# Borda/pyImSegm

Hardware: AMD Instinct MI355X
Metric: Mpixels/s end-to-end SLIC+fts+GC, 2048x2048 RGB; % HBM roofline (higher is better)
Workload: dtype f64; 1 GPU; single 2048x2048 RGB uint8 per GPU, SLIC(sp_size=46, K=2025, 10 sweeps) + colour mean/std/energy + 3-class alpha-expansion GC (gc_regul=2.0, edge=model), pre-fitted GMM, host numpy in -> segm int32 in host numpy (BASELINE configs[1]); bench_config=2, images_per_launch_chain=1, images_in_flight_per_gpu=4, hardware_queues=4, input_memory=pageable numpy, input_ring=default (one rank: measured in round 4), parallelism=images sharded over 1 GPU(s), 4 in flight per GPU (one HIP stream each)

## Files before the change

include/imsegm_hip.h:

```cpp
#ifndef IMSEGM_HIP_H
#define IMSEGM_HIP_H

#include <stddef.h>
#include <stdint.h>

#ifdef __cplusplus
extern "C" {
#endif

#define IMSEGM_API __attribute__((visibility("default")))

#define IMSEGM_U8 0
#define IMSEGM_F64 1
#define IMSEGM_F32 2

#define IMSEGM_E_FUSED_PATH (-3)

#define IMSEGM_E_FIT_CAPS (-4)

typedef struct imsegm_ctx imsegm_ctx;
typedef struct imsegm_image2d imsegm_image2d;

IMSEGM_API const char *imsegm_last_error(void);
IMSEGM_API int imsegm_version(void);
// ... 23 lines not shown
IMSEGM_API int imsegm_image2d_create(imsegm_ctx *ctx, int height, int width, imsegm_image2d **img_out);
IMSEGM_API void imsegm_image2d_destroy(imsegm_image2d *img);

IMSEGM_API int imsegm_image2d_upload(imsegm_image2d *img, const void *host_pixels, int dtype);

IMSEGM_API int imsegm_image2d_slic(imsegm_image2d *img, int minmax_normalize, int n_segments, double compactness,
                        const double *taps_z, int radius_z, const double *taps_y, int radius_y,
                        const double *taps_x, int radius_x, int max_iter, int enforce_connectivity,
                        double min_size_factor, double max_size_factor, int start_label,
                        int max_candidates, int slic_zero, int *n_labels_out);

IMSEGM_API int imsegm_image2d_get_labels(imsegm_image2d *img, int64_t *labels_out);
IMSEGM_API int imsegm_image2d_set_labels(imsegm_image2d *img, const int32_t *labels, int n_labels);
IMSEGM_API long imsegm_debug_conn_general_runs(void);
IMSEGM_API int imsegm_debug_slic_sweep_runs(long *persistent_runs_out, long *fallback_runs_out);
IMSEGM_API long imsegm_debug_gc_grid_fallbacks(void);
IMSEGM_API int imsegm_debug_exclusive_scan(const int32_t *host_in, int n, int32_t *host_out, int32_t *total);
IMSEGM_API int imsegm_image2d_enforce_connectivity(imsegm_image2d *img, const int32_t *labels, long min_size, long max_size,
                                                   int start_label, int *n_labels_out);
IMSEGM_API int imsegm_image2d_label_hist(imsegm_image2d *img, const int32_t *annot, int nb_annot, int64_t *hist_out);
IMSEGM_API int imsegm_image2d_get_lab(imsegm_image2d *img, double *lab_out);
IMSEGM_API int imsegm_image2d_get_nearest(imsegm_image2d *img, int32_t *nearest_out);
IMSEGM_API int imsegm_image2d_get_pre_scalars(imsegm_image2d *img, double out[3]);

IMSEGM_API int imsegm_image2d_color_stats(imsegm_image2d *img, double *mean_out, double *energy_out, double *var_out);

IMSEGM_API int imsegm_image2d_graph(imsegm_image2d *img, int32_t *edges_out, int edge_capacity, int *n_edges_out,
                         double *centres_out, uint8_t *present_out);

IMSEGM_API int imsegm_image2d_gather(imsegm_image2d *img, const int32_t *graph_labels, const double *proba,
// ... 219 lines not shown
```

pyimsegm_amd/_hip.py:

```python
import ctypes as C
import functools
import os
import threading

import numpy as np

_HERE = os.path.dirname(os.path.abspath(__file__))
LIB_PATH = os.environ.get('IMSEGM_HIP_LIBRARY') or os.path.join(_HERE, 'libimsegm_hip.so')

U8, F64, F32 = 0, 1, 2
PROFILE_GROUPS = {
    'slic_assign': 0,
    'slic': 1,
    'connectivity': 2,
    'color_stats': 3,
    'graph': 4,
    'graphcut': 5,
    'gather': 6,
    'slic_preprocess': 7,
    'terms': 8,
    'texture': 9,
}


# ... 68 lines not shown
    'imsegm_ctx_destroy': (None, [_vp]),
    'imsegm_ctx_synchronize': (C.c_int, [_vp]),
    'imsegm_ctx_profile_enable': (C.c_int, [_vp, C.c_int]),
    'imsegm_ctx_profile_reset': (C.c_int, [_vp]),
    'imsegm_ctx_profile_get': (C.c_int, [_vp, C.c_int, C.POINTER(C.c_double), _ip]),
    'imsegm_image2d_create': (C.c_int, [_vp, C.c_int, C.c_int, C.POINTER(_vp)]),
    'imsegm_image2d_destroy': (None, [_vp]),
    'imsegm_image2d_upload': (C.c_int, [_vp, _vp, C.c_int]),
    'imsegm_image2d_slic': (C.c_int, [_vp, C.c_int, C.c_int, C.c_double, _vp, C.c_int, _vp, C.c_int, _vp, C.c_int,
                                      C.c_int, C.c_int, C.c_double, C.c_double, C.c_int, C.c_int, C.c_int, _ip]),
    'imsegm_image2d_get_labels': (C.c_int, [_vp, _vp]),
    'imsegm_image2d_set_labels': (C.c_int, [_vp, _vp, C.c_int]),
    'imsegm_image2d_enforce_connectivity': (C.c_int, [_vp, _vp, C.c_long, C.c_long, C.c_int, _vp]),
    'imsegm_debug_conn_general_runs': (C.c_long, []),
    'imsegm_debug_slic_sweep_runs': (C.c_int, [_vp, _vp]),
    'imsegm_debug_gc_grid_fallbacks': (C.c_long, []),
    'imsegm_debug_exclusive_scan': (C.c_int, [_vp, C.c_int, _vp, _ip]),
    'imsegm_assume_bg_on_boundary': (C.c_int, [_vp, _vp, C.c_int, C.c_int, _vp, C.c_int, _ip]),
    'imsegm_image2d_all_finite': (C.c_int, [_vp, _ip]),
    'imsegm_image2d_lm_features': (C.c_int, [_vp, _vp, _vp, C.c_int, C.c_int, C.c_double, C.c_int, _vp]),
    'imsegm_batch2d_create': (C.c_int, [_vp, C.c_int, C.c_int, C.c_int, C.POINTER(_vp)]),
    'imsegm_batch2d_destroy': (None, [_vp]),
    'imsegm_batch2d_run_color': (C.c_int, [_vp, C.c_int, _vp, C.c_int, C.c_int, C.c_int, C.c_double, _vp, C.c_int, C.c_int, C.c_int,
                                           C.c_int, _vp, C.c_int, _vp, C.c_int, C.c_double, C.c_int, _vp, _vp, _vp]),
    'imsegm_batch2d_device_ptr': (C.c_int, [_vp, C.c_int, C.c_int, C.POINTER(_vp)]),
    'imsegm_device_pci_bus_id': (C.c_int, [C.c_int, C.c_char_p, C.c_int]),
    'imsegm_init': (C.c_int, [C.c_int]),
    'imsegm_debug_reload_env': (None, []),
    'imsegm_image2d_label_hist': (C.c_int, [_vp, _vp, C.c_int, _vp]),
    'imsegm_image2d_get_lab': (C.c_int, [_vp, _vp]),
# ... 1161 lines not shown


def exclusive_scan(values):
    values = np.ascontiguousarray(values, dtype=np.int32)
    out, total = np.empty_like(values), C.c_int(0)
    _check(load_library().imsegm_debug_exclusive_scan(values.ctypes.data, values.size, out.ctypes.data, C.byref(total)))
    return out, total.value


def slic_sweep_runs():
    a, b = C.c_long(0), C.c_long(0)
    _check(load_library().imsegm_debug_slic_sweep_runs(C.byref(a), C.byref(b)))
    return a.value, b.value


def assign_sweeps_per_launch(max_iter=10):
    persistent, fallback = slic_sweep_runs()
    return max_iter - 1 if (persistent > 0 and fallback == 0) else 1


def _device_array(sess, which, shape, typestr):
    ptr = _vp()
    _check(load_library().imsegm_image2d_device_ptr(sess._h, which, C.byref(ptr)))
    sess.ctx.synchronize()
    return DeviceArray(ptr.value, shape, typestr, sess)


def segm_device_array(sess):
    return _device_array(sess, 1, sess.shape, '<i4')

# ... 406 lines not shown
```

pyimsegm_amd/csrc/api.hip:

```cpp
#include "../../include/imsegm_hip.h"
#include "slic.h"

#include <atomic>
#include <cstdio>
#include <cstdlib>
#include <cstring>
#include <vector>

namespace imsegm {

static thread_local std::string g_error;

void set_error(const std::string &msg) { g_error = msg; }

bool hip_ok(hipError_t e, const char *what, const char *file, int line)
{
    if (e == hipSuccess) return true;
    char buf[512];
    snprintf(buf, sizeof(buf), "HIP error %d (%s) in `%s` at %s:%d", (int)e, hipGetErrorString(e), what, file, line);
    g_error = buf;
    return false;
}

static Knobs read_knobs()
{
    auto flag = [](const char *n) { return getenv(n) != nullptr; };
    auto num = [](const char *n, int dflt) { const char *e = getenv(n); return e ? atoi(e) : dflt; };
    Knobs k;
    k.slic_graph = flag("IMSEGM_SLIC_GRAPH");
    k.pre_3pass = flag("IMSEGM_PRE_3PASS");
    k.separate_finalize = flag("IMSEGM_SEPARATE_FINALIZE");
    k.fuse_finalize = flag("IMSEGM_FUSE_FINALIZE");
    k.conn_general = flag("IMSEGM_CONN_GENERAL");
    k.gc_no_topo_regs = flag("IMSEGM_GC_NO_TOPO_REGS");
    k.sep_wide_tile = flag("IMSEGM_SEP_WIDE_TILE");
    k.cc_merge_full = flag("IMSEGM_CC_MERGE_FULL");
    k.label_general = flag("IMSEGM_LABEL_GENERAL");
    k.terms_one_workgroup = flag("IMSEGM_TERMS_ONE_WORKGROUP");
    k.adjacency_table = flag("IMSEGM_ADJACENCY_TABLE");
    k.brick_cap = num("IMSEGM_BRICK_CAP", 0);
    k.gc_lds_level = num("IMSEGM_GC_LDS_LEVEL", 4);
    k.gc_threads = num("IMSEGM_GC_THREADS", 0);
    k.gc_grid_min_sites = num("IMSEGM_GC_GRID_MIN_SITES", 0);
    k.gc_grid_blocks = num("IMSEGM_GC_GRID_BLOCKS", 0);
    k.gc_one_workgroup = flag("IMSEGM_GC_ONE_WORKGROUP");
    k.gc_grid_test_absent = flag("IMSEGM_GC_GRID_TEST_ABSENT");
    k.fused_bitmap_mb = num("IMSEGM_FUSED_BITMAP_MB", 0);
// ... 252 lines not shown
    return 0;
}

long imsegm_debug_conn_general_runs(void) { return conn_general_runs(); }

void imsegm_debug_reload_env(void) { reload_knobs(); }

long imsegm_debug_gc_grid_fallbacks(void) { return gc_grid_fallbacks(); }

int imsegm_debug_slic_sweep_runs(long *persistent_runs_out, long *fallback_runs_out)
{
    slic_sweep_counters(persistent_runs_out, fallback_runs_out);
    return 0;
}

int imsegm_debug_exclusive_scan(const int32_t *host_in, int n, int32_t *host_out, int32_t *total)
{
    if (n < 0 || !total || (n > 0 && (!host_in || !host_out))) {
        set_error("exclusive_scan: n >= 0, and no null pointers");
        return -1;
    }
    int32_t *dev = nullptr;
    HIP_TRY(hipMalloc(&dev, ((size_t)n + 1) * sizeof(int32_t)));
    hipError_t e = n ? hipMemcpy(dev, host_in, (size_t)n * sizeof(int32_t), hipMemcpyHostToDevice) : hipSuccess;
    if (e == hipSuccess) {
        launch_exclusive_scan(dev, n, dev + n, nullptr);
        e = hipGetLastError();
    }
    if (e == hipSuccess && n) e = hipMemcpy(host_out, dev, (size_t)n * sizeof(int32_t), hipMemcpyDeviceToHost);
    if (e == hipSuccess) e = hipMemcpy(total, dev + n, sizeof(int32_t), hipMemcpyDeviceToHost);
// ... 49 lines not shown
```

pyimsegm_amd/csrc/api_image2d.hip:

```cpp
#include "session.h"

int slic_geometry(int H, int W, int n_segments, double compactness, int minmax_normalize, int max_candidates, int slic_zero,
                  SlicState &s, SlicGeometry &geo)
{
    long shape[3] = { 1, H, W };
    GridAxis ax[3];
    regular_grid3(shape, n_segments, ax);
    long ny = 0, nx = 0;
    for (long y = ax[1].start; y < H; y += ax[1].step) ny++;
    for (long x = ax[2].start; x < W; x += ax[2].step) nx++;
    const int K = (int)(ny * nx);
    if (K < 1) {
        set_error("slic: empty centroid grid");
        return -1;
    }
    double fsteps[3];
    for (int i = 0; i < 3; ++i) fsteps[i] = ax[i].all ? 1.0 : (double)ax[i].step;
    float step = (float)std::max(fsteps[0], std::max(fsteps[1], fsteps[2]));
    GridAxis axk[3];
    regular_grid3(shape, K, axk);
    memset(&s, 0, sizeof(s));
    s.H = H; s.W = W; s.K = K;
    s.step_y = axk[1].all ? 1 : (int)axk[1].step;
    s.step_x = axk[2].all ? 1 : (int)axk[2].step;
// ... 11 lines not shown
    s.slico = slic_zero ? 1 : 0;
    s.grid_y0 = (int)ax[1].start; s.grid_dy = (int)ax[1].step;
    s.grid_x0 = (int)ax[2].start; s.grid_dx = (int)ax[2].step; s.grid_nx = (int)nx;
    geo.K = K;
    geo.n_tiles = (size_t)cdiv(W, SLIC_TILE_X) * cdiv(H, SLIC_TILE_Y);
    return 0;
}

void slic_place_state(SlicState &s, const SlicGeometry &geo, unsigned char *cent, unsigned char *tiles, const double *premax, int *fail_host)
{
    const int K = geo.K;
    const size_t n_tiles = geo.n_tiles;
    s.premax = premax;
    unsigned char *cb = cent;
    s.acc = reinterpret_cast<long long *>(cb); cb += (size_t)K * 9 * 8;
    s.cy = reinterpret_cast<double *>(cb); cb += (size_t)K * 8;
    s.cx = reinterpret_cast<double *>(cb); cb += (size_t)K * 8;
    s.cL = reinterpret_cast<double *>(cb); cb += (size_t)K * 8;
    s.ca = reinterpret_cast<double *>(cb); cb += (size_t)K * 8;
    s.cb = reinterpret_cast<double *>(cb); cb += (size_t)K * 8;
    s.win = reinterpret_cast<int4 *>(cb); cb += (size_t)K * 16;
    s.mdc = reinterpret_cast<double *>(cb); cb += (size_t)K * 8;
    s.drift = reinterpret_cast<int *>(cb); cb += SLIC_DRIFT_SLOTS * sizeof(int);
    s.done = reinterpret_cast<int *>(cb); cb += (size_t)K * sizeof(int);
    s.fail_host = fail_host;
    s.tile_cands = reinterpret_cast<Cand *>(tiles);
    unsigned char *tb = tiles + n_tiles * SLIC_MAXC * sizeof(Cand);
    s.tile_rec = reinterpret_cast<Rec32 *>(tb); tb += n_tiles * SLIC_MAXC * sizeof(Rec32);
    s.tile_info = reinterpret_cast<TileInfo *>(tb); tb += n_tiles * sizeof(TileInfo);
    s.tile_k = reinterpret_cast<int *>(tb); tb += n_tiles * SLIC_MAXC * sizeof(int);
// ... 471 lines not shown
```

pyimsegm_amd/csrc/common.h:

```cpp
#pragma once
#include <hip/hip_runtime.h>
#include <stdint.h>
#include <string>
#include <type_traits>

#define IMSEGM_WAVE 64

namespace imsegm {

void set_error(const std::string &msg);
bool hip_ok(hipError_t e, const char *what, const char *file, int line);

#define HIP_TRY(expr)                                                                   \
    do {                                                                                \
        if (!::imsegm::hip_ok((expr), #expr, __FILE__, __LINE__)) return -1;            \
    } while (0)

struct Knobs {
    bool slic_graph, pre_3pass, separate_finalize, fuse_finalize, conn_general, gc_no_topo_regs,
        adjacency_table,
        cc_merge_full,
        terms_one_workgroup,
        label_general,
        sep_wide_tile;
    int brick_cap;
    int gc_lds_level;
    int gc_threads;
    int gc_grid_min_sites;
    int gc_grid_blocks;
    bool gc_one_workgroup;
    bool gc_grid_test_absent;
    int fused_bitmap_mb;
    std::string phase_dump;
};
// ... 400 lines not shown
```

pyimsegm_amd/csrc/session.h:

```cpp
#pragma once
#include "../../include/imsegm_hip.h"
#include "slic.h"

#include <atomic>
#include <cstdio>
#include <cstdlib>
#include <cstring>
#include <vector>

namespace imsegm {

struct DevBuf {
    void *p = nullptr;
    size_t cap = 0;
    int ensure(size_t bytes)
    {
        if (bytes <= cap) return 0;
        if (p) HIP_TRY(hipFree(p));
        p = nullptr;
        cap = 0;
        size_t want = bytes + bytes / 8 + 256;
        HIP_TRY(hipMalloc(&p, want));
        cap = want;
        return 0;
// ... 278 lines not shown
    size_t o_ref = 0, o_seg = 0, o_g = 0, o_d2 = 0, o_dist = 0, o_mask_a = 0, o_mask_b = 0, o_counts = 0, o_flags = 0, bytes = 0;
};
enum { BP_MASK = 0, BP_DISTANCE_MAP = 1, BP_DISTANCES = 2, BP_DISTANCES_SESSION = 3 };
BoundaryPlan boundary_plan(int H, int W, int kind);

}

struct SlicGeometry {
    int K;
    size_t n_tiles;
};
int slic_geometry(int H, int W, int n_segments, double compactness, int minmax_normalize, int max_candidates, int slic_zero,
                  imsegm::SlicState &s, SlicGeometry &geo);
void slic_place_state(imsegm::SlicState &s, const SlicGeometry &geo, unsigned char *cent, unsigned char *tiles, const double *premax,
                      int *fail_host);
inline size_t slic_cent_bytes(int K) { return (size_t)K * (5 * 8 + 16 + 9 * 8 + 16 + 4) + 256 + imsegm::SLIC_DRIFT_SLOTS * sizeof(int); }
inline size_t slic_tiles_bytes(size_t n_tiles, size_t n)
{
    return n_tiles * (imsegm::SLIC_MAXC * (sizeof(imsegm::Cand) + sizeof(imsegm::Rec32) + 2 * sizeof(int)) + sizeof(imsegm::TileInfo) + sizeof(int)) +
           n * 4 + 1024;
}
inline imsegm::ConnWork conn_work_from(int32_t *base_i32, size_t cap_bytes, uint8_t *base_u8, size_t n)
{
    imsegm::ConnWork w;
    int32_t *b = base_i32;
    w.parent = b; b += n;
    w.csize = b; b += n;
    w.newlabel = b; b += n;
    w.adjptr = b; b += n;
    w.queue = b; b += n;
    w.list = b; b += n;
// ... 15 lines not shown
```

pyimsegm_amd/csrc/slic.h:

```cpp
#pragma once
#include "common.h"
#include <algorithm>
#include <cfloat>
#include <cmath>

namespace imsegm {

enum { DT_U8 = 0, DT_F64 = 1, DT_F32 = 2 };

struct Taps {
    int r;
    double w[17];
};

constexpr int SLIC_TILE_X = 64, SLIC_TILE_Y = 32, SLIC_MAXC = 64;
struct Cand {
    double cy, cx, cL, ca, cb;
    int4 win;
    int k;
    float ry, rx;
    float fL, fa, fb;
    double mdc;
};

// ... 4 lines not shown
};
struct TileInfo {
    double ref[3];
    float Qy, Qx, QL, Qa, Qb;
    int count;
};

constexpr int SLIC_DRIFT_SLOTS = 64;
struct SlicState {
    int H, W, K;
    int step_y, step_x;
    double spatial_weight;
    double *cy, *cx, *cL, *ca, *cb;
    int4 *win;
    long long *acc;
    const double *premax;
    Cand *tile_cands;
    int *tile_count;
    Rec32 *tile_rec;
    TileInfo *tile_info;
    int *tile_k;
    uint32_t *tile_rows;
    int *leftover;
    int *leftover_count;
    int fast32;
    float kappa;
    int grid_y0, grid_dy, grid_x0, grid_dx, grid_nx;
    long long *phase_prof;
    int debug;
    int assign_units;
// ... 10 lines not shown
int launch_minmax(const void *src, int dtype, size_t n, unsigned long long *keys, double *out2, hipStream_t st, double *also_zero = nullptr,
                  ZBatch zb = ZBatch());
int launch_preprocess_color2d(const void *img, int dtype, int H, int W, int normalize, const double *minmax_dev,
                              const Taps &tz, const Taps &ty, const Taps &tx, double ratio, double *bufA,
                              double *bufB, double *premax_dev, hipStream_t st, bool premax_zeroed = false, ZBatch zb = ZBatch());
int launch_absmax_f64(const double *src, size_t n, double *out_dev, hipStream_t st);
struct ProfHook {
    void *user = nullptr;
    int (*begin)(void *, int) = nullptr;
    void (*end)(void *, int) = nullptr;
    void (*pair)(void *, int, hipEvent_t *, hipEvent_t *) = nullptr;
};
int slic_prepare_device();
void slic_sweep_counters(long *persistent_runs, long *fallback_runs);
void slic_sweep_note_fallback();
int launch_slic_iterations(SlicState s, const double *lab, const double *init_yx_dev, int32_t *labels, int max_iter,
                           int max_cand, const ProfHook &prof, hipStream_t st, bool *fused_update = nullptr, ZBatch zb = ZBatch());

struct VolState {
    int D, H, W, K;
    int step_z, step_y, step_x;
    double spatial_weight;
    double sz, sy, sx;
    double *cen;
    int *win;
    long long *acc;
    const double *premax;
    int grid_0[3], grid_d[3], grid_n[3];
    int nbz, nby, nbx;
    int brick_cap;
// ... 222 lines not shown
```

pyimsegm_amd/csrc/slic.hip:

```cpp
#include "slic.h"
#include <hip/hip_ext.h>
#include <atomic>
#include <cstdio>

namespace imsegm {

__device__ __forceinline__ int4 search_window(double cy, double cx, int step_y, int step_x, int H, int W)
{
    double a;
    int4 w;
    a = cy - (double)(2 * step_y);
    w.x = (int)(a > 0 ? a : 0.0);
    a = cy + (double)(2 * step_y);
    a = a + 1.0;
    w.y = (int)(a < (double)H ? a : (double)H);
    a = cx - (double)(2 * step_x);
    w.z = (int)(a > 0 ? a : 0.0);
    a = cx + (double)(2 * step_x);
    a = a + 1.0;
    w.w = (int)(a < (double)W ? a : (double)W);
    return w;
}

__device__ __forceinline__ void zshift_state(SlicState &s)
{
    const size_t zs = s.zs;
    ZSHIFT_NN(s.cy, zs); ZSHIFT_NN(s.cx, zs); ZSHIFT_NN(s.cL, zs); ZSHIFT_NN(s.ca, zs); ZSHIFT_NN(s.cb, zs);
    ZSHIFT_NN(s.win, zs); ZSHIFT_NN(s.acc, zs); ZSHIFT_NN(s.premax, zs);
    ZSHIFT_NN(s.tile_cands, zs); ZSHIFT_NN(s.tile_count, zs); ZSHIFT_NN(s.tile_rec, zs); ZSHIFT_NN(s.tile_info, zs); ZSHIFT_NN(s.tile_k, zs); ZSHIFT_NN(s.tile_rows, zs);
    ZSHIFT_NN(s.leftover, zs); ZSHIFT_NN(s.leftover_count, zs); ZSHIFT_NN(s.mdc, zs); ZSHIFT_NN(s.drift, zs); ZSHIFT(s.done, zs);
}

__global__ void k_centroid_init(SlicState s, const double *__restrict__ init_yx)
{
    zshift_state(s);
    int k = blockIdx.x * blockDim.x + threadIdx.x;
    if (k < SLIC_DRIFT_SLOTS) s.drift[k] = 0;
    if (k >= s.K) return;
    (void)init_yx;
    const int iy = k / s.grid_nx, ix = k - iy * s.grid_nx;
    double cy = (double)(s.grid_y0 + iy * s.grid_dy), cx = (double)(s.grid_x0 + ix * s.grid_dx);
    s.cy[k] = cy;
    s.cx[k] = cx;
    s.cL[k] = 0.0;
    s.ca[k] = 0.0;
    s.cb[k] = 0.0;
    s.win[k] = search_window(cy, cx, s.step_y, s.step_x, s.H, s.W);
    s.mdc[k] = 1.0;
    for (int j = 0; j < 9; ++j) s.acc[(size_t)k * 9 + j] = 0;
    if (s.done) s.done[k] = 0;
    if (k == 0) *s.leftover_count = 0;
}

__device__ __forceinline__ void centroid_finalize_one(const SlicState &s, int k, int drift_slot)
{
    if (k == 0) *s.leftover_count = 0;
    if (k >= s.K) return;
    long long *a = s.acc + (size_t)k * 9;
    long long n = a[0];
    if (n == 0) {
        s.win[k] = make_int4(0, 0, 0, 0);
    } else {
        double nn = (double)n;
        double cy = i64_to_double(a[1]) / nn;
        double cx = i64_to_double(a[2]) / nn;
        s.cy[k] = cy;
        s.cx[k] = cx;
        const double finv = ldexp(1.0, -fix_bits_of(*s.premax));
        s.cL[k] = fix_value(a[3], a[4], finv) / nn;
        s.ca[k] = fix_value(a[5], a[6], finv) / nn;
        s.cb[k] = fix_value(a[7], a[8], finv) / nn;
        s.win[k] = search_window(cy, cx, s.step_y, s.step_x, s.H, s.W);
        const int iy = k / s.grid_nx, ix = k - iy * s.grid_nx;
        const double dy = fabs(cy - (double)(s.grid_y0 + iy * s.grid_dy)), dx = fabs(cx - (double)(s.grid_x0 + ix * s.grid_dx));
        const int d = (int)ceil(fmax(dy, dx));
        if (d > 0) atomicMax(&s.drift[drift_slot], d);
    }
#pragma unroll
    for (int j = 0; j < 9; ++j) a[j] = 0;
}

__global__ void k_centroid_finalize(SlicState s, int drift_slot)
{
    zshift_state(s);
    centroid_finalize_one(s, blockIdx.x * blockDim.x + threadIdx.x, drift_slot);
}

constexpr int TILE_X = SLIC_TILE_X;
constexpr int TILE_Y = SLIC_TILE_Y;
constexpr int MAXC = SLIC_MAXC;

constexpr int BIN_TILES_PER_BLOCK = 4;
constexpr int BIN_MAX_K_LDS = 4096;
constexpr int BIN_LOCAL_MAX = 512;

__global__ void __launch_bounds__(256)
k_slic_bin(SlicState s, int tiles_x, int n_tiles, int max_cand, Cand *__restrict__ tile_cands,
           int *__restrict__ tile_count, int drift_slot)
{
    zshift_state(s);
    ZSHIFT(tile_cands, s.zs); ZSHIFT(tile_count, s.zs);
    extern __shared__ int4 lds_win[];
    __shared__ int ck[BIN_TILES_PER_BLOCK][MAXC];
    __shared__ float ckey[BIN_TILES_PER_BLOCK][MAXC];
    __shared__ float clb[BIN_TILES_PER_BLOCK][MAXC];
    const int lane = threadIdx.x & 63;
    const int wave = __builtin_amdgcn_readfirstlane(threadIdx.x >> 6);
    const int klds = min(s.K, BIN_MAX_K_LDS);
    const int drift = s.drift[drift_slot];
    const int reach_y = 2 * s.step_y + 1 + drift, reach_x = 2 * s.step_x + 1 + drift;
    const bool local = s.grid_dy > 0 && s.grid_dx > 0 && (long)(2 * reach_y + TILE_Y + 2 * s.grid_dy) * (2 * reach_x + TILE_X + 2 * s.grid_dx) <=
                       (long)BIN_LOCAL_MAX * s.grid_dy * s.grid_dx;
    if (!local) {
        for (int k = threadIdx.x; k < klds; k += 256) lds_win[k] = s.win[k];
        __syncthreads();
    }
    const int tile = blockIdx.x * BIN_TILES_PER_BLOCK + wave;
    if (tile >= n_tiles) return;
    const int tx0 = (tile % tiles_x) * TILE_X, ty0 = (tile / tiles_x) * TILE_Y;
    const int tx1 = min(tx0 + TILE_X, s.W), ty1 = min(ty0 + TILE_Y, s.H);
    int count = 0;
    int iy0 = 0, ix0 = 0, nry = 0, nrx = 1, total = s.K;
    if (local) {
        auto floor_div = [](int a, int b) { return a >= 0 ? a / b : -((-a + b - 1) / b); };
        const int ny = s.K / s.grid_nx;
        iy0 = max(0, floor_div(ty0 - reach_y - s.grid_y0 + s.grid_dy - 1, s.grid_dy));
        const int iy1 = min(ny - 1, floor_div(ty1 + reach_y - s.grid_y0, s.grid_dy));
        ix0 = max(0, floor_div(tx0 - reach_x - s.grid_x0 + s.grid_dx - 1, s.grid_dx));
        const int ix1 = min(s.grid_nx - 1, floor_div(tx1 + reach_x - s.grid_x0, s.grid_dx));
        nry = max(iy1 - iy0 + 1, 0);
        nrx = max(ix1 - ix0 + 1, 1);
        total = ix1 >= ix0 ? nry * nrx : 0;
    }
    for (int k0 = 0; k0 < total; k0 += 64) {
        int k = k0 + lane;
        bool hit = false;
        float key = 0.f;
        if (k < total) {
            int4 w;
            if (local) {
                const int jy = k / nrx;
                k = (iy0 + jy) * s.grid_nx + ix0 + (k - jy * nrx);
                w = s.win[k];
            } else {
                w = k < klds ? lds_win[k] : s.win[k];
            }
            hit = w.x < ty1 && w.y > ty0 && w.z < tx1 && w.w > tx0;
            float my = 0.5f * (float)(w.x + w.y) - 0.5f * (float)(ty0 + ty1);
            float mx = 0.5f * (float)(w.z + w.w) - 0.5f * (float)(tx0 + tx1);
            key = my * my + mx * mx;
        }
        unsigned long long m = __ballot(hit);
        if (hit) {
            int pos = count + __popcll(m & ((1ULL << lane) - 1ULL));
            if (pos < MAXC) {
                ck[wave][pos] = k;
                ckey[wave][pos] = key;
            }
        }
        count += __popcll(m);
    }
    __builtin_amdgcn_s_waitcnt(0);
    const bool overflow = count > max_cand;
    if (lane == 0) {
        tile_count[tile] = overflow ? -count : count;
        s.tile_info[tile].count = overflow ? -count : count;
    }
    if (overflow) return;
    const bool have = lane < count;
    const int k = have ? ck[wave][lane] : 0;
    Cand cd;
    cd.cy = s.cy[k]; cd.cx = s.cx[k]; cd.cL = s.cL[k]; cd.ca = s.ca[k]; cd.cb = s.cb[k];
    cd.win = s.win[k];
    cd.k = k;
    const double sw = s.spatial_weight;
    const double ryc = cd.cy - (double)(ty0 + 16), rxc = cd.cx - (double)(tx0 + 32);
    double dy = fmax(fmax(-16.0 - ryc, ryc - 15.0), 0.0), dx = fmax(fmax(-32.0 - rxc, rxc - 31.0), 0.0);
    const float lbt = __double2float_rd((dy * dy + dx * dx) * sw * 0.999999);
    const float key2 = have ? ckey[wave][lane] : 0.f;
    if (have) clb[wave][lane] = lbt;
    __builtin_amdgcn_s_waitcnt(0);
    __builtin_amdgcn_wave_barrier();
    int rank = 0;
    for (int j = 0; j < count; ++j) {
        const float kj = clb[wave][j], k2j = ckey[wave][j];
        rank += (kj < lbt) || (kj == lbt && (k2j < key2 || (k2j == key2 && j < lane)));
    }
    const unsigned long long first = __ballot(have && rank == 0);
// ... 778 lines not shown
                    s.cb[k] = fix_value(v[7], v[8], finv) / nn;
                    s.win[k] = search_window(cy, cx, s.step_y, s.step_x, s.H, s.W);
                    const int iy = k / s.grid_nx, ix = k - iy * s.grid_nx;
                    const double dy = fabs(cy - (double)(s.grid_y0 + iy * s.grid_dy)), dx = fabs(cx - (double)(s.grid_x0 + ix * s.grid_dx));
                    const int d = (int)ceil(fmax(dy, dx));
                    if (d > 0) atomicMax(&s.drift[s.drift_slot_next], d);
                }
#pragma unroll
                for (int j = 0; j < 9; ++j) s.acc[(size_t)k * 9 + j] = 0;
                s.done[k] = 0;
            }
        }
    }
}

static std::atomic<long> g_sweep_fallback{0};
void slic_sweep_counters(long *persistent_runs, long *fallback_runs)
{
    if (persistent_runs) *persistent_runs = 0;
    if (fallback_runs) *fallback_runs = g_sweep_fallback.load();
}
void slic_sweep_note_fallback() { g_sweep_fallback.fetch_add(1); }

int slic_prepare_device()
{
    static bool bin_attr[IMSEGM_MAX_DEVICES];
    int dev = 0;
    HIP_TRY(hipGetDevice(&dev));
    if (dev < 0 || dev >= IMSEGM_MAX_DEVICES || !bin_attr[dev]) {
        HIP_TRY(hipFuncSetAttribute((const void *)k_slic_bin, hipFuncAttributeMaxDynamicSharedMemorySize,
                                    BIN_MAX_K_LDS * (int)sizeof(int4)));
        if (dev >= 0 && dev < IMSEGM_MAX_DEVICES) bin_attr[dev] = true;
    }
    return 0;
}

int launch_slic_iterations(SlicState s, const double *lab, const double *init_yx_dev, int32_t *labels, int max_iter,
                           int max_cand, const ProfHook &prof, hipStream_t st, bool *fused_update, ZBatch zb)
{
    if (fused_update) *fused_update = false;
    s.zs = zb.zs;
    const unsigned nz = (unsigned)zb.nz;
    if (nz > 1 && (s.slico || s.phase_prof)) {
        set_error("slic: SLICO and the phase profiler do not take a batch");
        return -1;
    }
    const bool default_cand = max_cand <= 0 || max_cand >= MAXC;
    const bool env_separate_finalize = knobs().separate_finalize;
    const bool env_fuse_finalize = knobs().fuse_finalize;
    const long assign_workgroups = 2L * cdiv(s.W, TILE_X) * cdiv(s.H, TILE_Y);
    const bool fail_host_fuse = s.done != nullptr && s.fail_host != nullptr && !env_separate_finalize && default_cand &&
                                (env_fuse_finalize || assign_workgroups <= 1280);
    if (fail_host_fuse) *s.fail_host = 0;
    if (max_cand <= 0 || max_cand > MAXC) max_cand = MAXC;
    size_t n = (size_t)s.H * s.W;
    hipLaunchKernelGGL(k_centroid_init, dim3(cdiv(s.K, 256), 1, nz), 256, 0, st, s, init_yx_dev);
    dim3 grid(cdiv(s.W, TILE_X), 2 * cdiv(s.H, TILE_Y), nz);
    const int n_tiles = grid.x * cdiv(s.H, TILE_Y);
    const dim3 grid_tile(grid.x, cdiv(s.H, TILE_Y), nz);
    const int units = s.assign_units == 2 ? 2 : 1;
    if (slic_prepare_device()) return -1;
    bool grid_covers = false;
    {
        const int ny = s.K / s.grid_nx;
        const int reach_y = std::max(std::max(s.grid_y0, s.H - 1 - (s.grid_y0 + (ny - 1) * s.grid_dy)), s.grid_dy / 2 + 1);
        const int reach_x = std::max(std::max(s.grid_x0, s.W - 1 - (s.grid_x0 + (s.grid_nx - 1) * s.grid_dx)), s.grid_dx / 2 + 1);
        grid_covers = reach_y <= 2 * s.step_y && reach_x <= 2 * s.step_x;
    }
    if (!(max_iter > 0 && s.fast32 && s.spatial_weight > 1e-9 && grid_covers && !(s.debug & 32)))
        for (unsigned b = 0; b < nz; ++b)
            HIP_TRY(hipMemsetAsync(reinterpret_cast<unsigned char *>(labels) + (size_t)b * zb.zs, 0xff, n * sizeof(int32_t), st));
    static const bool print_occ = getenv("IMSEGM_PRINT_OCC") != nullptr;
    if (print_occ) {
        int nb = 0;
        HIP_TRY(hipOccupancyMaxActiveBlocksPerMultiprocessor(&nb, (const void *)k_slic_assign_dot<true, false, 1, false>, 256, 0));
        fprintf(stderr, "[occupancy] k_slic_assign_dot<true>: %d workgroups per CU\n", nb);
        HIP_TRY(hipOccupancyMaxActiveBlocksPerMultiprocessor(&nb, (const void *)k_slic_assign_dot<false, false, 1, false>, 256, 0));
        fprintf(stderr, "[occupancy] k_slic_assign_dot<false>: %d workgroups per CU\n", nb);
    }
    for (int it = 0; it < max_iter; ++it) {
        hipLaunchKernelGGL(k_slic_bin, dim3(cdiv(n_tiles, BIN_TILES_PER_BLOCK), 1, nz), 256,
                           (size_t)std::min(s.K, BIN_MAX_K_LDS) * sizeof(int4), st, s, (int)grid.x, n_tiles, max_cand,
                           s.tile_cands, s.tile_count, it % SLIC_DRIFT_SLOTS);
        const bool first = it == 0 && s.fast32 && s.spatial_weight > 1e-9;
        const bool dot = !first && s.fast32 && !s.slico && !(s.debug & 16);
        const bool first_grid = first && grid_covers && !(s.debug & 32);
        const bool accum = it + 1 < max_iter;
        const bool fuse = accum && s.done && fail_host_fuse && units == 1 && !s.phase_prof && (first_grid || dot);
        if (fuse && fused_update) *fused_update = true;
        SlicState sf = s;
        sf.fuse_finalize = fuse ? 1 : 0;
        sf.drift_slot_next = (it + 1) % SLIC_DRIFT_SLOTS;
        hipEvent_t ev_a = nullptr, ev_b = nullptr;
        if (prof.pair) prof.pair(prof.user, 0, &ev_a, &ev_b);
#define LAUNCH_ON(kernel, g, ...)                                                                                    \
    {                                                                                                                \
        if (ev_a) hipExtLaunchKernelGGL(kernel, g, dim3(256), 0, st, ev_a, ev_b, 0, __VA_ARGS__);                    \
        else hipLaunchKernelGGL(kernel, g, dim3(256), 0, st, __VA_ARGS__);                                           \
    }
#define LAUNCH_ASSIGN(kernel, ...) LAUNCH_ON(kernel, grid, __VA_ARGS__)
#define LAUNCH_DOT(ACC, FST)                                                                                         \
    {                                                                                                                \
        if (units == 2)                                                                                              \
            LAUNCH_ON((k_slic_assign_dot<ACC, FST, 2, false>), grid_tile, s, lab, labels, s.tile_cands, s.tile_rec, s.tile_info, s.tile_k) \
// ... 8 lines not shown
            if (accum) LAUNCH_DOT(true, false) else LAUNCH_DOT(false, false)
        } else if (first) {
            if (accum) LAUNCH_ASSIGN((k_slic_assign<true, true>), s, lab, labels, s.tile_cands, s.tile_count)
            else LAUNCH_ASSIGN((k_slic_assign<false, true>), s, lab, labels, s.tile_cands, s.tile_count)
        } else {
            SlicState se = s;
            if (s.slico) se.fast32 = 0;
            if (accum) LAUNCH_ASSIGN((k_slic_assign<true, false>), se, lab, labels, s.tile_cands, s.tile_count)
            else LAUNCH_ASSIGN((k_slic_assign<false, false>), se, lab, labels, s.tile_cands, s.tile_count)
        }
#undef LAUNCH_DOT
#undef LAUNCH_ON
#undef LAUNCH_ASSIGN
        if (it + 1 < max_iter) {
            if (!dot && !first_grid) hipLaunchKernelGGL(k_slic_leftover, dim3(64, 1, nz), 256, 0, st, s, lab, labels);
            if (!fuse) hipLaunchKernelGGL(k_centroid_finalize, dim3(cdiv(s.K, 256), 1, nz), 256, 0, st, s, (it + 1) % SLIC_DRIFT_SLOTS);
            if (s.slico)
                hipLaunchKernelGGL(k_slico_update, (int)std::min<size_t>(cdiv(n, (size_t)256), 4096), 256, 0, st, s, lab, labels);
        }
    }
    HIP_TRY(hipGetLastError());
    return 0;
}

}
```

Baseline: 6093 Mpixels/s.

## Compute SLIC centroids inside the bin kernel from double-buffered accumulator sums

Adds a templated k_slic_bin<true> path that reads raw per-cluster accumulator sums from the previous sweep, computes centroid position, colour and search window on the fly, and stages candidates in LDS. This removes the separate k_centroid_finalize launch and its global round-trip on each sweep. Accumulators are double-buffered (acc/acc2) so the bin kernel can zero the next buffer while reading the current one. Drift uses the previous slot plus a fixed slack, with a fail_host fallback flag. The path is enabled by default when there are more than 1280 assign workgroups, at the cost of redundant centroid computation across tiles and extra memory.

```diff
diff --git a/include/imsegm_hip.h b/include/imsegm_hip.h
--- a/include/imsegm_hip.h
+++ b/include/imsegm_hip.h
@@ -61,6 +61,7 @@
 IMSEGM_API int imsegm_image2d_set_labels(imsegm_image2d *img, const int32_t *labels, int n_labels);
 IMSEGM_API long imsegm_debug_conn_general_runs(void);
 IMSEGM_API int imsegm_debug_slic_sweep_runs(long *persistent_runs_out, long *fallback_runs_out);
+IMSEGM_API long imsegm_debug_slic_bin_sums_runs(void);
 IMSEGM_API long imsegm_debug_gc_grid_fallbacks(void);
 IMSEGM_API int imsegm_debug_exclusive_scan(const int32_t *host_in, int n, int32_t *host_out, int32_t *total);
 IMSEGM_API int imsegm_image2d_enforce_connectivity(imsegm_image2d *img, const int32_t *labels, long min_size, long max_size,
diff --git a/pyimsegm_amd/_hip.py b/pyimsegm_amd/_hip.py
--- a/pyimsegm_amd/_hip.py
+++ b/pyimsegm_amd/_hip.py
@@ -106,6 +106,7 @@
     'imsegm_image2d_enforce_connectivity': (C.c_int, [_vp, _vp, C.c_long, C.c_long, C.c_int, _vp]),
     'imsegm_debug_conn_general_runs': (C.c_long, []),
     'imsegm_debug_slic_sweep_runs': (C.c_int, [_vp, _vp]),
+    'imsegm_debug_slic_bin_sums_runs': (C.c_long, []),
     'imsegm_debug_gc_grid_fallbacks': (C.c_long, []),
     'imsegm_debug_exclusive_scan': (C.c_int, [_vp, C.c_int, _vp, _ip]),
     'imsegm_assume_bg_on_boundary': (C.c_int, [_vp, _vp, C.c_int, C.c_int, _vp, C.c_int, _ip]),
@@ -1297,6 +1298,10 @@
     return a.value, b.value
 
 
+def slic_bin_sums_runs():
+    return int(load_library().imsegm_debug_slic_bin_sums_runs())
+
+
 def assign_sweeps_per_launch(max_iter=10):
     persistent, fallback = slic_sweep_runs()
     return max_iter - 1 if (persistent > 0 and fallback == 0) else 1
diff --git a/pyimsegm_amd/csrc/api.hip b/pyimsegm_amd/csrc/api.hip
--- a/pyimsegm_amd/csrc/api.hip
+++ b/pyimsegm_amd/csrc/api.hip
@@ -31,6 +31,7 @@
     k.pre_3pass = flag("IMSEGM_PRE_3PASS");
     k.separate_finalize = flag("IMSEGM_SEPARATE_FINALIZE");
     k.fuse_finalize = flag("IMSEGM_FUSE_FINALIZE");
+    k.bin_from_sums = flag("IMSEGM_BIN_FROM_SUMS");
     k.conn_general = flag("IMSEGM_CONN_GENERAL");
     k.gc_no_topo_regs = flag("IMSEGM_GC_NO_TOPO_REGS");
     k.sep_wide_tile = flag("IMSEGM_SEP_WIDE_TILE");
@@ -313,6 +314,8 @@
     return 0;
 }
 
+long imsegm_debug_slic_bin_sums_runs(void) { return slic_bin_sums_runs(); }
+
 int imsegm_debug_exclusive_scan(const int32_t *host_in, int n, int32_t *host_out, int32_t *total)
 {
     if (n < 0 || !total || (n > 0 && (!host_in || !host_out))) {
diff --git a/pyimsegm_amd/csrc/api_image2d.hip b/pyimsegm_amd/csrc/api_image2d.hip
--- a/pyimsegm_amd/csrc/api_image2d.hip
+++ b/pyimsegm_amd/csrc/api_image2d.hip
@@ -49,6 +49,7 @@
     s.premax = premax;
     unsigned char *cb = cent;
     s.acc = reinterpret_cast<long long *>(cb); cb += (size_t)K * 9 * 8;
+    s.acc2 = reinterpret_cast<long long *>(cb); cb += (size_t)K * 9 * 8;
     s.cy = reinterpret_cast<double *>(cb); cb += (size_t)K * 8;
     s.cx = reinterpret_cast<double *>(cb); cb += (size_t)K * 8;
     s.cL = reinterpret_cast<double *>(cb); cb += (size_t)K * 8;
diff --git a/pyimsegm_amd/csrc/common.h b/pyimsegm_amd/csrc/common.h
--- a/pyimsegm_amd/csrc/common.h
+++ b/pyimsegm_amd/csrc/common.h
@@ -17,7 +17,7 @@
     } while (0)
 
 struct Knobs {
-    bool slic_graph, pre_3pass, separate_finalize, fuse_finalize, conn_general, gc_no_topo_regs,
+    bool slic_graph, pre_3pass, separate_finalize, fuse_finalize, bin_from_sums, conn_general, gc_no_topo_regs,
         adjacency_table,
         cc_merge_full,
         terms_one_workgroup,
diff --git a/pyimsegm_amd/csrc/session.h b/pyimsegm_amd/csrc/session.h
--- a/pyimsegm_amd/csrc/session.h
+++ b/pyimsegm_amd/csrc/session.h
@@ -316,7 +316,7 @@
                   imsegm::SlicState &s, SlicGeometry &geo);
 void slic_place_state(imsegm::SlicState &s, const SlicGeometry &geo, unsigned char *cent, unsigned char *tiles, const double *premax,
                       int *fail_host);
-inline size_t slic_cent_bytes(int K) { return (size_t)K * (5 * 8 + 16 + 9 * 8 + 16 + 4) + 256 + imsegm::SLIC_DRIFT_SLOTS * sizeof(int); }
+inline size_t slic_cent_bytes(int K) { return (size_t)K * (5 * 8 + 16 + 2 * 9 * 8 + 16 + 4) + 256 + imsegm::SLIC_DRIFT_SLOTS * sizeof(int); }
 inline size_t slic_tiles_bytes(size_t n_tiles, size_t n)
 {
     return n_tiles * (imsegm::SLIC_MAXC * (sizeof(imsegm::Cand) + sizeof(imsegm::Rec32) + 2 * sizeof(int)) + sizeof(imsegm::TileInfo) + sizeof(int)) +
diff --git a/pyimsegm_amd/csrc/slic.h b/pyimsegm_amd/csrc/slic.h
--- a/pyimsegm_amd/csrc/slic.h
+++ b/pyimsegm_amd/csrc/slic.h
@@ -42,6 +42,7 @@
     double *cy, *cx, *cL, *ca, *cb;
     int4 *win;
     long long *acc;
+    long long *acc2;
     const double *premax;
     Cand *tile_cands;
     int *tile_count;
@@ -82,6 +83,7 @@
 int slic_prepare_device();
 void slic_sweep_counters(long *persistent_runs, long *fallback_runs);
 void slic_sweep_note_fallback();
+long slic_bin_sums_runs();
 int launch_slic_iterations(SlicState s, const double *lab, const double *init_yx_dev, int32_t *labels, int max_iter,
                            int max_cand, const ProfHook &prof, hipStream_t st, bool *fused_update = nullptr, ZBatch zb = ZBatch());
 
diff --git a/pyimsegm_amd/csrc/slic.hip b/pyimsegm_amd/csrc/slic.hip
--- a/pyimsegm_amd/csrc/slic.hip
+++ b/pyimsegm_amd/csrc/slic.hip
@@ -26,7 +26,7 @@
 {
     const size_t zs = s.zs;
     ZSHIFT_NN(s.cy, zs); ZSHIFT_NN(s.cx, zs); ZSHIFT_NN(s.cL, zs); ZSHIFT_NN(s.ca, zs); ZSHIFT_NN(s.cb, zs);
-    ZSHIFT_NN(s.win, zs); ZSHIFT_NN(s.acc, zs); ZSHIFT_NN(s.premax, zs);
+    ZSHIFT_NN(s.win, zs); ZSHIFT_NN(s.acc, zs); ZSHIFT_NN(s.acc2, zs); ZSHIFT_NN(s.premax, zs);
     ZSHIFT_NN(s.tile_cands, zs); ZSHIFT_NN(s.tile_count, zs); ZSHIFT_NN(s.tile_rec, zs); ZSHIFT_NN(s.tile_info, zs); ZSHIFT_NN(s.tile_k, zs); ZSHIFT_NN(s.tile_rows, zs);
     ZSHIFT_NN(s.leftover, zs); ZSHIFT_NN(s.leftover_count, zs); ZSHIFT_NN(s.mdc, zs); ZSHIFT_NN(s.drift, zs); ZSHIFT(s.done, zs);
 }
@@ -35,7 +35,7 @@
 {
     zshift_state(s);
     int k = blockIdx.x * blockDim.x + threadIdx.x;
-    if (k < SLIC_DRIFT_SLOTS) s.drift[k] = 0;
+    if (k < SLIC_DRIFT_SLOTS) s.drift[k] = k == 0 ? max(s.step_y, s.step_x) / 4 + 1 : 0;
     if (k >= s.K) return;
     (void)init_yx;
     const int iy = k / s.grid_nx, ix = k - iy * s.grid_nx;
@@ -48,8 +48,35 @@
     s.win[k] = search_window(cy, cx, s.step_y, s.step_x, s.H, s.W);
     s.mdc[k] = 1.0;
     for (int j = 0; j < 9; ++j) s.acc[(size_t)k * 9 + j] = 0;
+    for (int j = 0; j < 9; ++j) s.acc2[(size_t)k * 9 + j] = 0;
     if (s.done) s.done[k] = 0;
     if (k == 0) *s.leftover_count = 0;
+}
+
+struct CentroidYX {
+    double cy, cx;
+    int4 win;
+    int d;
+};
+__device__ __forceinline__ CentroidYX centroid_position(const SlicState &s, int k, long long n, long long sum_y, long long sum_x)
+{
+    CentroidYX c;
+    const double nn = (double)n;
+    c.cy = i64_to_double(sum_y) / nn;
+    c.cx = i64_to_double(sum_x) / nn;
+    c.win = search_window(c.cy, c.cx, s.step_y, s.step_x, s.H, s.W);
+    const int iy = k / s.grid_nx, ix = k - iy * s.grid_nx;
+    const double dy = fabs(c.cy - (double)(s.grid_y0 + iy * s.grid_dy)), dx = fabs(c.cx - (double)(s.grid_x0 + ix * s.grid_dx));
+    c.d = (int)ceil(fmax(dy, dx));
+    return c;
+}
+__device__ __forceinline__ void centroid_colour(const SlicState &s, long long n, const long long *a, double &cL, double &ca, double &cb)
+{
+    const double nn = (double)n;
+    const double finv = ldexp(1.0, -fix_bits_of(*s.premax));
+    cL = fix_value(a[3], a[4], finv) / nn;
+    ca = fix_value(a[5], a[6], finv) / nn;
+    cb = fix_value(a[7], a[8], finv) / nn;
 }
 
 __device__ __forceinline__ void centroid_finalize_one(const SlicState &s, int k, int drift_slot)
@@ -61,20 +88,16 @@
     if (n == 0) {
         s.win[k] = make_int4(0, 0, 0, 0);
     } else {
-        double nn = (double)n;
-        double cy = i64_to_double(a[1]) / nn;
-        double cx = i64_to_double(a[2]) / nn;
-        s.cy[k] = cy;
-        s.cx[k] = cx;
-        const double finv = ldexp(1.0, -fix_bits_of(*s.premax));
-        s.cL[k] = fix_value(a[3], a[4], finv) / nn;
-        s.ca[k] = fix_value(a[5], a[6], finv) / nn;
-        s.cb[k] = fix_value(a[7], a[8], finv) / nn;
-        s.win[k] = search_window(cy, cx, s.step_y, s.step_x, s.H, s.W);
-        const int iy = k / s.grid_nx, ix = k - iy * s.grid_nx;
-        const double dy = fabs(cy - (double)(s.grid_y0 + iy * s.grid_dy)), dx = fabs(cx - (double)(s.grid_x0 + ix * s.grid_dx));
-        const int d = (int)ceil(fmax(dy, dx));
-        if (d > 0) atomicMax(&s.drift[drift_slot], d);
+        const CentroidYX c = centroid_position(s, k, n, a[1], a[2]);
+        s.cy[k] = c.cy;
+        s.cx[k] = c.cx;
+        double cL, ca, cb;
+        centroid_colour(s, n, a, cL, ca, cb);
+        s.cL[k] = cL;
+        s.ca[k] = ca;
+        s.cb[k] = cb;
+        s.win[k] = c.win;
+        if (c.d > 0) atomicMax(&s.drift[drift_slot], c.d);
     }
 #pragma unroll
     for (int j = 0; j < 9; ++j) a[j] = 0;
@@ -93,7 +116,9 @@
 constexpr int BIN_TILES_PER_BLOCK = 4;
 constexpr int BIN_MAX_K_LDS = 4096;
 constexpr int BIN_LOCAL_MAX = 512;
-
+__device__ __forceinline__ int bin_drift_slack(const SlicState &s) { return max(s.step_y, s.step_x); }
+
+template <bool SUMS>
 __global__ void __launch_bounds__(256)
 k_slic_bin(SlicState s, int tiles_x, int n_tiles, int max_cand, Cand *__restrict__ tile_cands,
            int *__restrict__ tile_count, int drift_slot)
@@ -101,17 +126,25 @@
     zshift_state(s);
     ZSHIFT(tile_cands, s.zs); ZSHIFT(tile_count, s.zs);
     extern __shared__ int4 lds_win[];
+    __shared__ double ccy[SUMS ? BIN_TILES_PER_BLOCK : 1][SUMS ? MAXC : 1], ccx[SUMS ? BIN_TILES_PER_BLOCK : 1][SUMS ? MAXC : 1];
+    __shared__ int4 cwin[SUMS ? BIN_TILES_PER_BLOCK : 1][SUMS ? MAXC : 1];
+    __shared__ double ccol[SUMS ? BIN_TILES_PER_BLOCK : 1][3][SUMS ? MAXC : 1];
+    if (SUMS) {
+        const size_t words = (size_t)s.K * 9;
+        for (size_t i = (size_t)blockIdx.x * 256 + threadIdx.x; i < words; i += (size_t)gridDim.x * 256) s.acc2[i] = 0;
+    }
     __shared__ int ck[BIN_TILES_PER_BLOCK][MAXC];
     __shared__ float ckey[BIN_TILES_PER_BLOCK][MAXC];
     __shared__ float clb[BIN_TILES_PER_BLOCK][MAXC];
     const int lane = threadIdx.x & 63;
     const int wave = __builtin_amdgcn_readfirstlane(threadIdx.x >> 6);
     const int klds = min(s.K, BIN_MAX_K_LDS);
-    const int drift = s.drift[drift_slot];
+    const int drift_prev = SUMS ? s.drift[(drift_slot + SLIC_DRIFT_SLOTS - 1) % SLIC_DRIFT_SLOTS] : 0;
+    const int drift = SUMS ? drift_prev + bin_drift_slack(s) : s.drift[drift_slot];
     const int reach_y = 2 * s.step_y + 1 + drift, reach_x = 2 * s.step_x + 1 + drift;
     const bool local = s.grid_dy > 0 && s.grid_dx > 0 && (long)(2 * reach_y + TILE_Y + 2 * s.grid_dy) * (2 * reach_x + TILE_X + 2 * s.grid_dx) <=
                        (long)BIN_LOCAL_MAX * s.grid_dy * s.grid_dx;
-    if (!local) {
+    if (!SUMS && !local) {
         for (int k = threadIdx.x; k < klds; k += 256) lds_win[k] = s.win[k];
         __syncthreads();
     }
@@ -119,7 +152,7 @@
     if (tile >= n_tiles) return;
     const int tx0 = (tile % tiles_x) * TILE_X, ty0 = (tile / tiles_x) * TILE_Y;
     const int tx1 = min(tx0 + TILE_X, s.W), ty1 = min(ty0 + TILE_Y, s.H);
-    int count = 0;
+    int count = 0, home_d = 0;
     int iy0 = 0, ix0 = 0, nry = 0, nrx = 1, total = s.K;
     if (local) {
         auto floor_div = [](int a, int b) { return a >= 0 ? a / b : -((-a + b - 1) / b); };
@@ -132,6 +165,69 @@
         nrx = max(ix1 - ix0 + 1, 1);
         total = ix1 >= ix0 ? nry * nrx : 0;
     }
+    if (SUMS) {
+        auto node_of = [&](int j) {
+            if (!local) return j;
+            const int jy = j / nrx;
+            return (iy0 + jy) * s.grid_nx + ix0 + (j - jy * nrx);
+        };
+        auto load_sums = [&](int k, long long (&v)[9]) {
+#pragma unroll
+            for (int j = 0; j < 9; ++j) v[j] = 0;
+            if (k >= 0) {
+                const long long *a = s.acc + (size_t)k * 9;
+#pragma unroll
+                for (int j = 0; j < 9; ++j) v[j] = a[j];
+            }
+        };
+        long long v[9], vn[9];
+        int k = lane < total ? node_of(lane) : -1;
+        load_sums(k, v);
+        for (int k0 = 0; k0 < total; k0 += 64) {
+            const int kn = k0 + 64 + lane < total ? node_of(k0 + 64 + lane) : -1;
+            load_sums(kn, vn);
+            bool hit = false;
+            float key = 0.f;
+            double cy = 0.0, cx = 0.0, cL = 0.0, ca = 0.0, cb = 0.0;
+            int4 w = make_int4(0, 0, 0, 0);
+            if (k >= 0) {
+                const long long n = v[0];
+                const int gy = k / s.grid_nx, gx = k - gy * s.grid_nx;
+                const int ny_ = min(max(s.grid_y0 + gy * s.grid_dy, 0), s.H - 1), nx_ = min(max(s.grid_x0 + gx * s.grid_dx, 0), s.W - 1);
+                const bool home = ny_ >= ty0 && ny_ < ty1 && nx_ >= tx0 && nx_ < tx1;
+                if (n != 0) {
+                    const CentroidYX c = centroid_position(s, k, n, v[1], v[2]);
+                    cy = c.cy; cx = c.cx; w = c.win;
+                    centroid_colour(s, n, v, cL, ca, cb);
+                    if (local && c.d > drift) *reinterpret_cast<volatile int *>(s.fail_host) = 1;
+                    if (home) {
+                        s.cy[k] = cy; s.cx[k] = cx; s.cL[k] = cL; s.ca[k] = ca; s.cb[k] = cb;
+                        home_d = max(home_d, c.d);
+                    }
+                }
+                if (home) s.win[k] = w;
+                hit = w.x < ty1 && w.y > ty0 && w.z < tx1 && w.w > tx0;
+                float my = 0.5f * (float)(w.x + w.y) - 0.5f * (float)(ty0 + ty1);
+                float mx = 0.5f * (float)(w.z + w.w) - 0.5f * (float)(tx0 + tx1);
+                key = my * my + mx * mx;
+            }
+            unsigned long long m = __ballot(hit);
+            if (hit) {
+                int pos = count + __popcll(m & ((1ULL << lane) - 1ULL));
+                if (pos < MAXC) {
+                    ck[wave][pos] = k;
+                    ckey[wave][pos] = key;
+                    ccy[wave][pos] = cy; ccx[wave][pos] = cx;
+                    ccol[wave][0][pos] = cL; ccol[wave][1][pos] = ca; ccol[wave][2][pos] = cb;
+                    cwin[wave][pos] = w;
+                }
+            }
+            count += __popcll(m);
+            k = kn;
+#pragma unroll
+            for (int j = 0; j < 9; ++j) v[j] = vn[j];
+        }
+    } else
     for (int k0 = 0; k0 < total; k0 += 64) {
         int k = k0 + lane;
         bool hit = false;
@@ -160,6 +256,15 @@
         }
         count += __popcll(m);
     }
+    if (SUMS) {
+#pragma unroll
+        for (int off = 32; off > 0; off >>= 1) home_d = max(home_d, __shfl_xor(home_d, off, 64));
+        if (lane == 0 && tile == 0 && drift_prev > 0) atomicMax(&s.drift[drift_slot], drift_prev);
+        if (lane == 0 && home_d > drift_prev &&
+            home_d > __hip_atomic_load(&s.drift[drift_slot], __ATOMIC_RELAXED, __HIP_MEMORY_SCOPE_AGENT))
+            atomicMax(&s.drift[drift_slot], home_d);
+        if (lane == 0 && tile == 0) *s.leftover_count = 0;
+    }
     __builtin_amdgcn_s_waitcnt(0);
     const bool overflow = count > max_cand;
     if (lane == 0) {
@@ -170,8 +275,18 @@
     const bool have = lane < count;
     const int k = have ? ck[wave][lane] : 0;
     Cand cd;
-    cd.cy = s.cy[k]; cd.cx = s.cx[k]; cd.cL = s.cL[k]; cd.ca = s.ca[k]; cd.cb = s.cb[k];
-    cd.win = s.win[k];
+    if (SUMS) {
+        cd.cy = cd.cx = cd.cL = cd.ca = cd.cb = 0.0;
+        cd.win = make_int4(0, 0, 0, 0);
+        if (have) {
+            cd.cy = ccy[wave][lane]; cd.cx = ccx[wave][lane];
+            cd.cL = ccol[wave][0][lane]; cd.ca = ccol[wave][1][lane]; cd.cb = ccol[wave][2][lane];
+            cd.win = cwin[wave][lane];
+        }
+    } else {
+        cd.cy = s.cy[k]; cd.cx = s.cx[k]; cd.cL = s.cL[k]; cd.ca = s.ca[k]; cd.cb = s.cb[k];
+        cd.win = s.win[k];
+    }
     cd.k = k;
     const double sw = s.spatial_weight;
     const double ryc = cd.cy - (double)(ty0 + 16), rxc = cd.cx - (double)(tx0 + 32);
@@ -980,7 +1095,8 @@
     }
 }
 
-static std::atomic<long> g_sweep_fallback{0};
+static std::atomic<long> g_sweep_fallback{0}, g_sweep_bin_sums{0};
+long slic_bin_sums_runs() { return g_sweep_bin_sums.load(); }
 void slic_sweep_counters(long *persistent_runs, long *fallback_runs)
 {
     if (persistent_runs) *persistent_runs = 0;
@@ -994,7 +1110,7 @@
     int dev = 0;
     HIP_TRY(hipGetDevice(&dev));
     if (dev < 0 || dev >= IMSEGM_MAX_DEVICES || !bin_attr[dev]) {
-        HIP_TRY(hipFuncSetAttribute((const void *)k_slic_bin, hipFuncAttributeMaxDynamicSharedMemorySize,
+        HIP_TRY(hipFuncSetAttribute((const void *)k_slic_bin<false>, hipFuncAttributeMaxDynamicSharedMemorySize,
                                     BIN_MAX_K_LDS * (int)sizeof(int4)));
         if (dev >= 0 && dev < IMSEGM_MAX_DEVICES) bin_attr[dev] = true;
     }
@@ -1017,7 +1133,13 @@
     const long assign_workgroups = 2L * cdiv(s.W, TILE_X) * cdiv(s.H, TILE_Y);
     const bool fail_host_fuse = s.done != nullptr && s.fail_host != nullptr && !env_separate_finalize && default_cand &&
                                 (env_fuse_finalize || assign_workgroups <= 1280);
-    if (fail_host_fuse) *s.fail_host = 0;
+    const bool bin_sums = s.done != nullptr && s.fail_host != nullptr && !env_separate_finalize && default_cand && !env_fuse_finalize &&
+                          (knobs().bin_from_sums || assign_workgroups > 1280) && s.assign_units != 2 && !s.phase_prof && s.fast32 &&
+                          !s.slico && !(s.debug & 16);
+    if (fail_host_fuse || bin_sums) *s.fail_host = 0;
+    long long *const acc_block[2] = { s.acc, s.acc2 };
+    bool counted = false;
+    bool deferred_prev = false;
     if (max_cand <= 0 || max_cand > MAXC) max_cand = MAXC;
     size_t n = (size_t)s.H * s.W;
     hipLaunchKernelGGL(k_centroid_init, dim3(cdiv(s.K, 256), 1, nz), 256, 0, st, s, init_yx_dev);
@@ -1045,15 +1167,29 @@
         fprintf(stderr, "[occupancy] k_slic_assign_dot<false>: %d workgroups per CU\n", nb);
     }
     for (int it = 0; it < max_iter; ++it) {
-        hipLaunchKernelGGL(k_slic_bin, dim3(cdiv(n_tiles, BIN_TILES_PER_BLOCK), 1, nz), 256,
-                           (size_t)std::min(s.K, BIN_MAX_K_LDS) * sizeof(int4), st, s, (int)grid.x, n_tiles, max_cand,
-                           s.tile_cands, s.tile_count, it % SLIC_DRIFT_SLOTS);
+        if (bin_sums) s.acc = acc_block[it & 1];
+        if (deferred_prev) {
+            SlicState sb = s;
+            sb.acc = acc_block[(it - 1) & 1];
+            sb.acc2 = acc_block[it & 1];
+            hipLaunchKernelGGL(k_slic_bin<true>, dim3(cdiv(n_tiles, BIN_TILES_PER_BLOCK), 1, nz), 256, 0, st, sb, (int)grid.x, n_tiles,
+                               max_cand, s.tile_cands, s.tile_count, it % SLIC_DRIFT_SLOTS);
+        } else {
+            hipLaunchKernelGGL(k_slic_bin<false>, dim3(cdiv(n_tiles, BIN_TILES_PER_BLOCK), 1, nz), 256,
+                               (size_t)std::min(s.K, BIN_MAX_K_LDS) * sizeof(int4), st, s, (int)grid.x, n_tiles, max_cand,
+                               s.tile_cands, s.tile_count, it % SLIC_DRIFT_SLOTS);
+        }
         const bool first = it == 0 && s.fast32 && s.spatial_weight > 1e-9;
         const bool dot = !first && s.fast32 && !s.slico && !(s.debug & 16);
         const bool first_grid = first && grid_covers && !(s.debug & 32);
         const bool accum = it + 1 < max_iter;
-        const bool fuse = accum && s.done && fail_host_fuse && units == 1 && !s.phase_prof && (first_grid || dot);
+        const bool fuse = accum && s.done && fail_host_fuse && !bin_sums && units == 1 && !s.phase_prof && (first_grid || dot);
         if (fuse && fused_update) *fused_update = true;
+        const bool defer = accum && bin_sums && (first_grid || dot);
+        if (defer && !counted) g_sweep_bin_sums.fetch_add(1);
+        counted = counted || defer;
+        if (defer && fused_update) *fused_update = true;
+        deferred_prev = defer;
         SlicState sf = s;
         sf.fuse_finalize = fuse ? 1 : 0;
         sf.drift_slot_next = (it + 1) % SLIC_DRIFT_SLOTS;
@@ -1092,7 +1228,7 @@
 #undef LAUNCH_ASSIGN
         if (it + 1 < max_iter) {
             if (!dot && !first_grid) hipLaunchKernelGGL(k_slic_leftover, dim3(64, 1, nz), 256, 0, st, s, lab, labels);
-            if (!fuse) hipLaunchKernelGGL(k_centroid_finalize, dim3(cdiv(s.K, 256), 1, nz), 256, 0, st, s, (it + 1) % SLIC_DRIFT_SLOTS);
+            if (!fuse && !defer) hipLaunchKernelGGL(k_centroid_finalize, dim3(cdiv(s.K, 256), 1, nz), 256, 0, st, s, (it + 1) % SLIC_DRIFT_SLOTS);
             if (s.slico)
                 hipLaunchKernelGGL(k_slico_update, (int)std::min<size_t>(cdiv(n, (size_t)256), 4096), 256, 0, st, s, lab, labels);
         }
```

Measured after the change: 5870 Mpixels/s. 0.963x the previous value.
